# zju3dv/RelightableAvatar

Hardware: AMD Instinct MI355X
Metric: rays_per_sec (higher is better)
Workload: dtype f16

## Files before the change

relightableavatar_amd/csrc/ra_api.cpp:

```cpp
#include "ra_api_impl.hpp"
#include <cmath>

int check_ready(ra_ctx* c, const char* who) {
    if (!c) { ra_set_error(std::string(who) + ": null ctx"); return 1; }
    if (!c->have_weights) { ra_set_error(std::string(who) + ": weights not finalized"); return 1; }
    if (!c->have_frame) { ra_set_error(std::string(who) + ": no frame set (ra_set_frame)"); return 1; }
    if (hipSetDevice(c->device) != hipSuccess) { ra_set_error(std::string(who) + ": hipSetDevice failed"); return 1; }
    return 0;
}

static void zero_chunk_counters(ra_ctx* c, hipStream_t s) {
    hipMemsetAsync(icnt(c, 0), 0, CNT_ALL * sizeof(int), s);
    c->fc_next = 0;
    c->fc_wrapped = false;
    c->cnt_zero = true;
}
int* next_fine_counter(ra_ctx* c, hipStream_t s) {
    if (c->fc_next >= CNT_FC_SLOTS) {
        hipMemsetAsync(icnt(c, CNT_FC0), 0, CNT_FC_SLOTS * sizeof(int), s);
        c->fc_next = 0;
        c->fc_wrapped = true;
    }
    return icnt(c, CNT_FC0 + c->fc_next++);
}
// ... 329 lines not shown
    return 0;
}

struct LvisStage {
    const float *surf, *norm_slots, *acc, *bbox;
    const int *hit_idx, *hit_count;
    int P, no_visibility, local_visibility;
    float near_offset;
    const ra_trace_params* shadow;
    int n_boxes;
    const float* boxes;
    const int *box_start, *pix_nn, *perm;
    bool split_wide_groups;
    float *lvis, *ldot;
};
static int light_visibility_stage(ra_ctx* c, LvisStage& st, hipStream_t s) {
    const int P = st.P;
    const ra_trace_params& shadow = *st.shadow;
    int err = 0;
    const int L = c->n_lights;
    const size_t NR = (size_t)P * L;
    st.lvis = c->buf<float>("lv_lvis", NR, &err);
    st.ldot = c->buf<float>("lv_ldot", NR, &err);
    ShadowGen g{};
    g.surf = st.surf; g.norm = st.norm_slots; g.acc = st.acc; g.hit_idx = st.hit_idx; g.hit_count = st.hit_count; g.ldir = c->light_dir.as<float>();
    for (int k = 0; k < 6; ++k) g.bbox[k] = st.bbox[k];
    g.n_boxes = st.n_boxes > 1 ? st.n_boxes : 0;
    for (int j = 0; j < g.n_boxes; ++j) {
        for (int k = 0; k < 6; ++k) g.boxes[j][k] = st.boxes[6 * j + k];
        g.box_start[j] = st.box_start[j];
    }
    if (g.n_boxes) g.box_start[g.n_boxes] = st.box_start[g.n_boxes];
    g.perm = g.n_boxes ? st.perm : nullptr;
    g.near_offset = st.near_offset; g.L = L; g.no_visibility = st.no_visibility; g.local_visibility = st.local_visibility;
    g.split_wide_groups = st.split_wide_groups ? 1 : 0;
    g.lvis = st.lvis; g.ldot = st.ldot;
    g.ray_count = icnt(c, CNT_RAYS);
    const bool traced = !(st.no_visibility || st.local_visibility);
    TraceState sh{};
    float* ssdf = nullptr;
    if (traced) {
        g.ray_pix = c->buf<int>("lv_pix", NR, &err);
        g.ray_light = c->buf<int>("lv_light", NR, &err);
        g.ray_slot = c->buf<int>("lv_slot", NR, &err);
        g.near_ = c->buf<float>("lv_near", NR, &err);
        g.far_ = c->buf<float>("lv_far", NR, &err);
        sh = alloc_trace(c, "sh_", (int)NR, shadow.soft_shadow != 0, &err);
        ssdf = c->buf<float>("sh_sdf", NR, &err);
    }
    const bool keyed = traced && key_tier(c) && c->key_valid;
    const size_t NK = keyed ? (size_t)P * (size_t)(L < KEY_LIGHTS_MAX ? L : KEY_LIGHTS_MAX) : 0;
    if (err) return 1;
    if (c->gate && c->gate->armed) RA_HIP(hipStreamWaitEvent(s, c->gate->done, 0));
    launch_shadow_gen(g, P, s, c->cnt_zero);
    c->cnt_zero = false;
    if (traced) {
        sh.near_ = g.near_; sh.far_ = g.far_; sh.tan_i = c->light_sharp.as<float>(); sh.light = g.ray_light;
        launch_trace_init(sh, (int)NR, g.ray_count, shadow, s);
        RaySet r2{};
        r2.mode = 2; r2.o = st.surf; r2.t = sh.t; r2.pix = g.ray_pix; r2.light = g.ray_light; r2.ldir = c->light_dir.as<float>();
        r2.n_dev = g.ray_count;
        r2.skip = c->cfg.query_skip ? sh.stuck : nullptr;
        r2.nn_hint = c->buf<int>("lv_nn", NR * 3, &err);
        if (err) return 1;
        for (int it = 0; it < shadow.iters; ++it) {
            r2.hint_valid = it > 0;
            r2.hint_src = it == 0 ? st.pix_nn : nullptr;
            r2.hint_src_index = it == 0 ? g.ray_pix : nullptr;
            if (hdq_pass(c, r2, (int)NR, shadow.dist_th, 1, ssdf, s, Q_OTHER, keyed ? c->key_mask.as<unsigned char>() : nullptr, (int)NK)) return 1;
            launch_trace_update(sh, ssdf, (int)NR, g.ray_count, it, shadow, s);
        }
        launch_shadow_scatter(sh.occ, g.ray_slot, g.ray_count, (int)NR, st.lvis, s);
        launch_accumulate(g.ray_count, &dcnt(c)->n_shadow_rays, s);
    }
    if (c->gate) { RA_HIP(hipEventRecord(c->gate->done, s)); c->gate->armed = true; }
    return 0;
}

int ra_begin_render(ra_ctx* c) {
    RA_CHECK(c, "ra_begin_render: null ctx");
    c->call_no = 0;
    return 0;
}

int ra_set_key_probes(ra_ctx* c, const float* probes, int n, int ph, int pw, int accumulate, void* stream) {
    RA_CHECK(c && n >= 0 && (n == 0 || (probes && ph > 0 && pw > 0)), "ra_set_key_probes: bad arguments");
    if (n == 0) { c->key_external = false; c->key_valid = false; return 0; }
    RA_CHECK(c->have_weights && c->n_lights > 0, "ra_set_key_probes: needs the relight network's light set (ra_finalize_weights)");
    RA_HIP(hipSetDevice(c->device));
    const bool acc = accumulate && c->key_external && c->key_valid;
    c->key_external = true;
    if (!key_tier(c)) { c->key_valid = false; return 0; }
    if (c->key_mask.ensure((size_t)c->n_lights) || c->key_share.ensure((size_t)c->n_lights * sizeof(float))) return 1;
    launch_key_lights(probes, n, ph, pw, c->light_dir.as<float>(), c->light_area.as<float>(), c->n_lights, c->cfg.key_light_share, KEY_LIGHTS_MAX,
                      acc ? 1 : 0, c->key_share.as<float>(), c->key_mask.as<unsigned char>(), (hipStream_t)stream);
    c->key_valid = true;
    RA_HIP(hipGetLastError());
    return 0;
}

static int sort_hits(ra_ctx* c, const char* who, const float* surf, const float* acc, int P, const float* bbox, int* hit_idx, hipStream_t s) {
    int err = 0;
    const size_t tb = sort_hits_temp_bytes(P);
    unsigned* k0 = c->buf<unsigned>("hs_k0", P, &err);
    unsigned* k1 = c->buf<unsigned>("hs_k1", P, &err);
    int* v0 = c->buf<int>("hs_v0", P, &err);
    char* tmp = c->buf<char>("hs_tmp", tb + 16, &err);
    if (err) return 1;
    if (launch_sort_hits(surf, acc, P, bbox, k0, k1, v0, hit_idx, tmp, tb, s)) { ra_set_error(std::string(who) + ": radix sort failed"); return 1; }
    return 0;
}
static int sort_rays(ra_ctx* c, const char* who, const float** ray_o, const float** ray_d, const float** near_, const float** far_, int P,
                     const float* bbox, const int** perm, hipStream_t s) {
    int err = 0;
    const size_t tb = sort_hits_temp_bytes(P);
    unsigned* k0 = c->buf<unsigned>("hs_k0", P, &err);
    unsigned* k1 = c->buf<unsigned>("hs_k1", P, &err);
    int* v0 = c->buf<int>("hs_v0", P, &err);
    int* pm = c->buf<int>("rs_perm", P, &err);
    char* tmp = c->buf<char>("hs_tmp", tb + 16, &err);
    float* so = c->buf<float>("rs_o", (size_t)P * 3, &err);
    float* sd = c->buf<float>("rs_d", (size_t)P * 3, &err);
    float* sn = c->buf<float>("rs_n", P, &err);
    float* sf = c->buf<float>("rs_f", P, &err);
    if (err) return 1;
    const int rc = bbox ? launch_sort_rays(*ray_o, *ray_d, *near_, *far_, P, bbox, k0, k1, v0, pm, tmp, tb, so, sd, sn, sf, s)
// ... 261 lines not shown
```

relightableavatar_amd/csrc/ra_kernels.hpp:

```cpp
#pragma once
#include "ra_common.hpp"
#include "ra_lpips_pack.hpp"

struct RaySet {
    int mode;
    const float* x;
    const float* o;
    const float* d;
    const float* t;
    const int* pix;
    const int* light;
    const float* ldir;
    const int* n_dev;
    const unsigned char* skip;
    int* nn_hint;
    int hint_valid;
    const int* hint_src;
    const int* hint_src_index;
};

struct HdqOut {
    float* sdf;
    int* fine_count;
    int* fine_idx;
// ... 28 lines not shown
struct TraceState {
    float *t, *d0, *dt, *st, *ot, *cd, *occ, *off, *rlx;
    const float *near_, *far_;
    const float* tan_i;
    const int* light;
    unsigned char* stuck;
};
void launch_trace_init(const TraceState& ts, int n, const int* n_dev, const ra_trace_params& p, hipStream_t s);

void launch_trace_update(const TraceState& ts, const float* sdf, int n, const int* n_dev, int iter,
                         const ra_trace_params& p, hipStream_t s);

void launch_surface_finish(const float* ray_o, const float* ray_d, const float* st, const float* occ, int P, float* surf,
                           float* depth, float* acc, int* hit_idx, int* hit_count, hipStream_t s, int* slot_of_ray = nullptr,
                           bool counter_is_zero = false);
void launch_slot_index(const int* hit_idx, const int* hit_count, int P, int* slot_of_ray, hipStream_t s);
struct MapJob { const float* src; float* dst; int C; int premul; int src_full; };
constexpr int RA_MAX_MAP_JOBS = 16;
struct EmitMaps { MapJob job[RA_MAX_MAP_JOBS]; long long end[RA_MAX_MAP_JOBS]; int n_jobs; const int* slot_of_ray; const float* acc; const int* perm; int P; };
void launch_emit_maps(const EmitMaps& m, hipStream_t s);
void launch_surface_samples(const float* surf, const float* ray_d, const int* hit_idx, const int* hit_count, int P, int S,
                            float range, float* x, float* v, int* n_out, hipStream_t s);
struct SurfaceMaps {
    float *cpts, *bpts, *resd, *norm, *albedo, *rough, *rgb;
    float* valbedo;
};
void launch_surface_composite(const float* raw, int C, int S, const int* hit_count, int P, int relight, const ra_config& cfg,
                              const SurfaceMaps& m, hipStream_t s);

constexpr int RA_MAX_BOXES = 32;
struct ShadowGen {
    const float* surf;
    const float* norm;
    const float* acc;
    const int* hit_idx;
    const int* hit_count;
    const float* ldir;
    float bbox[6];
    int n_boxes;
    float boxes[RA_MAX_BOXES][6];
    int box_start[RA_MAX_BOXES + 1];
    const int* perm;
    float near_offset;
    int L;
    int no_visibility, local_visibility;
    int split_wide_groups;
    float* lvis;
    float* ldot;
    int* ray_pix;
    int* ray_light;
    int* ray_slot;
    float *near_, *far_;
    int* ray_count;
};
void launch_key_lights(const float* probes, int n, int ph, int pw, const float* ldir, const float* area, int L, float share, int kmax,
                       int accumulate, float* smax, unsigned char* key, hipStream_t s);
void launch_gather_shard_rays(const long long* idx, int n, const float* ro, const float* rd, const float* nr, const float* fr, float* so, float* sd,
                              float* sn, float* sf, hipStream_t s);
void launch_scatter_rows(const float* src, const long long* src_idx, const long long* dst_idx, long long n, int C, float* dst, hipStream_t s);
void launch_shadow_gen(const ShadowGen& g, int P, hipStream_t s, bool counter_is_zero = false);
void launch_debug_aabb(const float* o, const float* d, int n, const float* bbox6, float* nr, float* fr, hipStream_t s);
void launch_debug_brdf(const float* p2l, const float* p2c, const float* nrm, const float* alb, const float* rough, int L, int N, const ra_config& cfg,
                       float* out, hipStream_t s);
size_t sort_hits_temp_bytes(int P);
int launch_sort_hits(const float* surf, const float* acc, int P, const float* bbox_min, unsigned* keys_in, unsigned* keys_out,
                     int* vals_in, int* hit_idx_out, void* temp, size_t temp_bytes, hipStream_t s);
void launch_shadow_scatter(const float* occ, const int* ray_slot, const int* ray_count, int max_rays, float* lvis, hipStream_t s);

struct ShadeIn {
    const float* ray_o;
    const float* surf;
    const int* idx;
    const int* count;
    int n;
    const float *norm, *albedo, *rough;
    const float *lvis, *ldot;
    const float *light_xyz, *light_area;
    int L;
    const float* probes;
    int n_probes, ph, pw;
    int want_spec;
    float *rgb, *shade, *spec;
};
void launch_shade(const ShadeIn& in, const ra_config& cfg, hipStream_t s);

constexpr int SHADE_BWD_MAX_GRID = 768;
constexpr size_t SHADE_BWD_LDS_BYTES = 65536;
struct ShadeBwd {
    const float *ray_o, *surf, *norm, *albedo, *rough;
    const float* lvis;
    const float *light_xyz, *light_area; int L;
    const float* probes; int n_probes, ph, pw;
    const float* d_rgb;
    int P;
    float *d_albedo, *d_rough, *d_probes;
    float* slabs;
};
int shade_bwd_grid(int P);
int shade_bwd_probes_per_launch(int ph, int pw);
void launch_shade_bwd(const ShadeBwd& a, const ra_config& cfg, hipStream_t s);

constexpr int HEADS_PARAMS = 99332;
constexpr int HEADS_MAX_GRID = 128;
constexpr int HEADS_CHUNK = 32768;
constexpr size_t HEADS_TAPE_BYTES_PER_TILE = 163840;
constexpr size_t HEADS_W16_BYTES = 2 * 66048 * 2;
struct HeadsIO {
    const float *theta, *feat;
    int n;
    float *albedo, *rough;
    const float *d_albedo, *d_rough;
    float* d_theta;
    void* w16;
    unsigned* amax;
    void* tape;
    float* slabs;
};
int heads_grid(int n);
void launch_heads_forward(const HeadsIO& io, const ra_config& cfg, hipStream_t s);
void launch_heads_backward(const HeadsIO& io, const ra_config& cfg, hipStream_t s);
// ... 240 lines not shown
```

relightableavatar_amd/csrc/ra_trace.hip:

```cpp
#include "ra_kernels.hpp"
#include "ra_shade_dev.hpp"
#include <hipcub/hipcub.hpp>

namespace {

constexpr int TPB = 256;

__device__ __forceinline__ int live_count(const int* n_dev, int n) { return n_dev ? min(*n_dev, n) : n; }

__device__ __forceinline__ float linspace01(int s, int S) {
    if (S == 1) return 0.f;
    const float step = 1.f / (float)(S - 1);
    return (s < S / 2) ? (float)s * step : 1.f - (float)(S - 1 - s) * step;
}

__global__ void trace_init_kernel(TraceState ts, int n_launch, const int* n_dev, float offset, float relax) {
    const int i = blockIdx.x * TPB + threadIdx.x;
    if (i >= live_count(n_dev, n_launch)) return;
    const float nr = ts.near_[i], fr = ts.far_[i];
    ts.t[i] = nr;
    ts.d0[i] = 1e9f;
    ts.occ[i] = 1.f;
    if (ts.stuck) ts.stuck[i] = 0;
    if (ts.dt) ts.dt[i] = 1e9f;
    if (ts.st) ts.st[i] = fr;
    if (ts.ot) ts.ot[i] = fr;
    if (ts.cd) ts.cd[i] = 1e9f;
    if (ts.off) ts.off[i] = offset;
    if (ts.rlx) ts.rlx[i] = relax;
}

template <bool SOFT>
__global__ void trace_update_kernel(TraceState ts, const float* __restrict__ sdf, int n_launch, const int* n_dev, int iter,
                                    ra_trace_params p) {
    const int i = blockIdx.x * TPB + threadIdx.x;
    if (i >= live_count(n_dev, n_launch)) return;
    const float d1 = sdf[i];
    const float d0 = ts.d0[i];
    float t = ts.t[i];
    const float t_prev = t;
    float occ = ts.occ[i];
    const float nr = ts.near_[i], fr = ts.far_[i];
    float tan_i = p.tan_i;
    if (SOFT) {
        const float ti = ts.tan_i ? (ts.light ? ts.tan_i[ts.light[i]] : ts.tan_i[i]) : p.tan_i;
        tan_i = p.tan_i_multiplier * ti;
    }
    const float tan2 = (1.f / tan_i) * 2.f;
    float off = ts.off ? ts.off[i] : p.offset;
    float rlx = ts.rlx ? ts.rlx[i] : p.relax;
    float ot = ts.ot ? ts.ot[i] : 0.f;
    if (SOFT && p.clay_book && iter >= p.shadow_skip_iter) {
        const float dx0 = d0 + rlx * d0 + off;
        const float dx1 = d1 + rlx * d1 + off;
        const float dy = (dx1 * dx1) / (2.f * dx0);
        const float dx = (sqrtf(dx1 * dx1 - dy * dy) - off) / (1.f + rlx);
        const float den = fmaxf(fmaxf(t - dy, nr), p.eps);
        const float cls = fmaxf(dx, 0.f) / den / tan2;
        const bool msk = (cls < occ) && (dy < t) && (dx1 > 0.f) && (dx0 > 0.f) && (dx > 0.f) && (dy > 0.f) && (dy < dx0);
        if (msk) { ot = t - dy; occ = cls; }
    }
    if (iter >= p.shadow_skip_iter) {
        const float cls = fmaxf(d1, 0.f) / fmaxf(fmaxf(t, nr), p.eps) / tan2;
        if (cls < occ) { ot = t; occ = cls; }
    }
    if (!SOFT) {
        const float d1u = fabsf(d1), d0u = fabsf(d0);
        float st = ts.st[i], cd = ts.cd[i];
        const float dt = ts.dt[i];
        const float s0 = (d0 > 0.f) ? 1.f : ((d0 < 0.f) ? -1.f : 0.f);
        const float s1 = (d1 > 0.f) ? 1.f : ((d1 < 0.f) ? -1.f : 0.f);
        if (s0 != s1) {
            st = t - dt * fminf(fmaxf(d1u / (d0u + d1u + p.eps), 0.f), 1.f);
            off = 0.f;
            rlx = 0.f;
        }
        if (d1u < cd) { cd = d1u; st = t; }
        ts.st[i] = st;
        ts.cd[i] = cd;
        ts.off[i] = off;
        ts.rlx[i] = rlx;
    }
    const float dtn = d1 + rlx * d1 + off;
    t = t + dtn;
    t = fminf(t, fr);
    t = fmaxf(t, nr);
    if (ts.dt) ts.dt[i] = dtn;
    ts.t[i] = t;
    if (ts.stuck) ts.stuck[i] = (t == t_prev || (SOFT && occ == 0.f)) ? 1 : 0;
    ts.d0[i] = d1;
    ts.occ[i] = occ;
    if (ts.ot) ts.ot[i] = ot;
}

__global__ void surface_finish_kernel(const float* __restrict__ ro, const float* __restrict__ rd, const float* __restrict__ st,
                                      const float* __restrict__ occ, int P, float* __restrict__ surf, float* __restrict__ depth,
                                      float* __restrict__ acc, int* __restrict__ hit_idx, int* __restrict__ hit_count, int* __restrict__ slot_of_ray) {
    const int i = blockIdx.x * TPB + threadIdx.x;
    bool hit = false;
    if (i < P) {
        if (slot_of_ray) slot_of_ray[i] = -1;
        const float s = st[i];
        const float sx = ro[3 * i] + s * rd[3 * i], sy = ro[3 * i + 1] + s * rd[3 * i + 1], sz = ro[3 * i + 2] + s * rd[3 * i + 2];
        surf[3 * i] = sx; surf[3 * i + 1] = sy; surf[3 * i + 2] = sz;
        depth[i] = (sx - ro[3 * i]) / rd[3 * i];
        const float a = 1.f - occ[i];
        acc[i] = a;
        hit = a > 0.f;
    }
    const unsigned long long m = __ballot(hit);
    if (m == 0ull) return;
    const int lane = threadIdx.x & 63;
    int base = 0;
    if (lane == 0) base = atomicAdd(hit_count, __popcll(m));
    base = __shfl(base, 0);
    if (hit) hit_idx[base + __popcll(m & ((1ull << lane) - 1ull))] = i;
}

__device__ __forceinline__ unsigned expand10t(unsigned v) {
    v = (v * 0x00010001u) & 0xFF0000FFu;
    v = (v * 0x00000101u) & 0x0F00F00Fu;
    v = (v * 0x00000011u) & 0xC30C30C3u;
    v = (v * 0x00000005u) & 0x49249249u;
    return v;
}

__global__ void hit_keys_kernel(const float* __restrict__ surf, const float* __restrict__ acc, int P, float bx, float by, float bz,
                                unsigned* __restrict__ keys, int* __restrict__ vals) {
    const int i = blockIdx.x * TPB + threadIdx.x;
    if (i >= P) return;
    unsigned k = 0xffffffffu;
    if (acc[i] > 0.f) {
        const unsigned qx = (unsigned)fminf(fmaxf((surf[3 * i] - bx) * 256.f, 0.f), 1023.f);
        const unsigned qy = (unsigned)fminf(fmaxf((surf[3 * i + 1] - by) * 256.f, 0.f), 1023.f);
        const unsigned qz = (unsigned)fminf(fmaxf((surf[3 * i + 2] - bz) * 256.f, 0.f), 1023.f);
        k = (expand10t(qx) << 2) | (expand10t(qy) << 1) | expand10t(qz);
    }
    keys[i] = k;
    vals[i] = i;
}

__global__ void ray_keys_kernel(const float* __restrict__ ro, const float* __restrict__ rd, const float* __restrict__ nr, int P,
                                float bx, float by, float bz, const float* __restrict__ origin_dev, unsigned* __restrict__ keys,
                                int* __restrict__ vals) {
    const int i = blockIdx.x * TPB + threadIdx.x;
// ... 211 lines not shown
            if (g.no_visibility) lv = 1.f;
            else if (g.local_visibility) lv = ldot > 0.f ? 1.f : 0.f;
            else {
                const bool front = (ldot > 0.f) && (acc > 0.f);
                lv = 0.f;
                if (front) {
                    const float d[3] = {dx, dy, dz};
                    aabb_near_far(box, o, d, nr, fr);
                    nr = fmaxf(nr, g.near_offset);
                    fr = fmaxf(fr, g.near_offset);
                    trace = nr < fr;
                    lv = 1.f;
                }
            }
            t_ldot[lane][ll] = ldot;
            t_lvis[lane][ll] = lv;
        }
        nrv[round] = nr; frv[round] = fr;
        if (trace) tmask |= 1u << round;
        const unsigned long long m = __ballot(trace);
        if (lane == 0) { cnt[0][ll] = __popcll(m & 0xffffffffull); cnt[1][ll] = __popcll(m >> 32); }
    }
    __syncthreads();
    if (threadIdx.x == 0) {
        int tot = 0;
        if (halves) {
            for (int hf = 0; hf < 2; ++hf)
                for (int k = 0; k < NL; ++k) { const int c = cnt[hf][k]; cnt[hf][k] = tot; tot += c; }
        } else {
            for (int k = 0; k < NL; ++k) {
                const int c0 = cnt[0][k], c1 = cnt[1][k];
                cnt[0][k] = tot; cnt[1][k] = tot + c0; tot += c0 + c1;
            }
        }
        cnt[0][NL] = tot ? atomicAdd(g.ray_count, tot) : 0;
    }
    __syncthreads();
    const int gbase = cnt[0][NL];
#pragma unroll
    for (int round = 0; round < ROUNDS; ++round) {
        const int ll = round * (TPB / 64) + wv;
        const bool trace = (tmask >> round) & 1u;
        const unsigned long long m = __ballot(trace);
        if (trace) {
            const int hf = lane >> 5;
            const unsigned mh = hf ? (unsigned)(m >> 32) : (unsigned)m;
            const int s = gbase + cnt[hf][ll] + __popc(mh & ((1u << (lane & 31)) - 1u));
            const int l = lc * SG_LIGHTS + ll;
            g.ray_pix[s] = r;
            g.ray_light[s] = l;
            g.ray_slot[s] = h * g.L + l;
            g.near_[s] = nrv[round];
            g.far_[s] = frv[round];
        }
    }
    const int col = threadIdx.x & (SG_LIGHTS - 1), l = lc * SG_LIGHTS + col;
    for (int row = threadIdx.x / SG_LIGHTS; row < 64; row += TPB / SG_LIGHTS) {
        const int hh = grp * 64 + row;
        if (hh < nh && l < g.L) {
            g.ldot[(size_t)hh * g.L + l] = t_ldot[row][col];
            g.lvis[(size_t)hh * g.L + l] = t_lvis[row][col];
        }
    }
}

__global__ void shadow_scatter_kernel(const float* __restrict__ occ, const int* __restrict__ ray_slot, const int* __restrict__ ray_count,
                                      int max_rays, float* __restrict__ lvis) {
    const int i = blockIdx.x * TPB + threadIdx.x;
    if (i >= min(*ray_count, max_rays)) return;
    lvis[ray_slot[i]] = occ[i];
}

__global__ __launch_bounds__(TPB) void key_lights_kernel(const float* __restrict__ probes, int n, int ph, int pw, const float* __restrict__ ldir,
                                                         const float* __restrict__ area, int L, float share, int kmax, int accumulate,
                                                         float* __restrict__ smax, unsigned char* __restrict__ key) {
    extern __shared__ float kl_w[];
    __shared__ float red[TPB / 64];
    for (int q = 0; q < n; ++q) {
        const float* img = probes + (size_t)q * ph * pw * 3;
        float part = 0.f;
        for (int l = threadIdx.x; l < L; l += TPB) {
            const float d[3] = {ldir[3 * l], ldir[3 * l + 1], ldir[3 * l + 2]};
            float c[3];
            sample_probe(img, ph, pw, d, c);
            float w = (c[0] + c[1] + c[2]) * (1.f / 3.f) * area[l];
            w = w > 0.f ? w : 0.f;
            kl_w[l] = w;
            part += w;
        }
#pragma unroll
        for (int sh = 32; sh > 0; sh >>= 1) part += __shfl_xor(part, sh);
        if ((threadIdx.x & 63) == 0) red[threadIdx.x >> 6] = part;
        __syncthreads();
        float total = 0.f;
#pragma unroll
        for (int k = 0; k < TPB / 64; ++k) total += red[k];
        for (int l = threadIdx.x; l < L; l += TPB) {
            const float sh_l = total > 0.f ? kl_w[l] / total : 0.f;
            smax[l] = (q == 0 && !accumulate) ? sh_l : fmaxf(smax[l], sh_l);
        }
        __syncthreads();
    }
    for (int l = threadIdx.x; l < L; l += TPB) kl_w[l] = smax[l];
    __syncthreads();
    const float thr = fmaxf(share, 4.f / (float)L);
    for (int l = threadIdx.x; l < L; l += TPB) {
        const float w = kl_w[l];
        bool cand = w >= thr;
        if (cand) {
            int rank = 0;
            for (int j = 0; j < L; ++j) rank += (kl_w[j] > w) || (kl_w[j] == w && j < l);
            cand = rank < kmax;
        }
        key[l] = (unsigned char)cand;
    }
}

__global__ void debug_brdf_kernel(const float* __restrict__ p2l, const float* __restrict__ p2c, const float* __restrict__ nrm, const float* __restrict__ alb,
                                  const float* __restrict__ rough, int L, int N, ra_config cfg, float* __restrict__ out) {
    const int i = blockIdx.x * TPB + threadIdx.x;
    if (i >= L * N) return;
// ... 187 lines not shown
    __syncthreads();
    float pre = 1.f;
    for (int k = 0; k < g; ++k) pre *= tseg[k][j];
#pragma unroll
    for (int c = 0; c < 15; ++c) part[g][c][j] = o[c] * pre;
    part[g][15][j] = acc * pre;
    part[g][16][j] = depth * pre;
    __syncthreads();
    if (blockIdx.x * 64 + j >= P) return;
    const int w_ = perm ? perm[r] : r;
    float a_ = 0.f;
#pragma unroll
    for (int k = 0; k < VC_SEG; ++k) a_ += part[k][15][j];
    if (g == 15) {
        float d_ = 0.f;
#pragma unroll
        for (int k = 0; k < VC_SEG; ++k) d_ += part[k][16][j];
        if (out.acc) out.acc[w_] = a_;
        if (out.depth) out.depth[w_] = d_;
        return;
    }
    float v = 0.f;
#pragma unroll
    for (int k = 0; k < VC_SEG; ++k) v += part[k][g][j];
    v += (1.f - a_) * bg;
    float* dst = g < 3 ? out.cpts : (g < 6 ? out.bpts : (g < 9 ? out.resd : (g < 12 ? out.norm : out.rgb)));
    if (dst) dst[3 * w_ + g % 3] = v;
}

inline dim3 grid_for(long long n) { return dim3((unsigned)((n + TPB - 1) / TPB)); }

}

void launch_debug_aabb(const float* o, const float* d, int n, const float* bbox6, float* nr, float* fr, hipStream_t s) {
    if (n <= 0) return;
    Box6 b; for (int k = 0; k < 6; ++k) b.v[k] = bbox6[k];
    hipLaunchKernelGGL(debug_aabb_kernel, grid_for(n), dim3(TPB), 0, s, o, d, n, b, nr, fr);
}

void launch_debug_brdf(const float* p2l, const float* p2c, const float* nrm, const float* alb, const float* rough, int L, int N, const ra_config& cfg,
                       float* out, hipStream_t s) {
    if (L * N <= 0) return;
    hipLaunchKernelGGL(debug_brdf_kernel, grid_for((long long)L * N), dim3(TPB), 0, s, p2l, p2c, nrm, alb, rough, L, N, cfg, out);
}

void launch_trace_init(const TraceState& ts, int n, const int* n_dev, const ra_trace_params& p, hipStream_t s) {
    if (n <= 0) return;
    hipLaunchKernelGGL(trace_init_kernel, grid_for(n), dim3(TPB), 0, s, ts, n, n_dev, p.offset, p.relax);
}

void launch_trace_update(const TraceState& ts, const float* sdf, int n, const int* n_dev, int iter, const ra_trace_params& p,
                         hipStream_t s) {
    if (n <= 0) return;
    if (p.soft_shadow) hipLaunchKernelGGL(trace_update_kernel<true>, grid_for(n), dim3(TPB), 0, s, ts, sdf, n, n_dev, iter, p);
    else hipLaunchKernelGGL(trace_update_kernel<false>, grid_for(n), dim3(TPB), 0, s, ts, sdf, n, n_dev, iter, p);
}

void launch_surface_finish(const float* ray_o, const float* ray_d, const float* st, const float* occ, int P, float* surf,
                           float* depth, float* acc, int* hit_idx, int* hit_count, hipStream_t s, int* slot_of_ray, bool counter_is_zero) {
    if (!counter_is_zero) hipMemsetAsync(hit_count, 0, sizeof(int), s);
    if (P <= 0) return;
    hipLaunchKernelGGL(surface_finish_kernel, grid_for(P), dim3(TPB), 0, s, ray_o, ray_d, st, occ, P, surf, depth, acc, hit_idx, hit_count, slot_of_ray);
}

void launch_slot_index(const int* hit_idx, const int* hit_count, int P, int* slot_of_ray, hipStream_t s) {
    if (P <= 0) return;
    hipLaunchKernelGGL(slot_index_kernel, grid_for(P), dim3(TPB), 0, s, hit_idx, hit_count, slot_of_ray);
}

void launch_emit_maps(const EmitMaps& m, hipStream_t s) {
    if (m.n_jobs <= 0 || m.P <= 0) return;
    hipLaunchKernelGGL(emit_maps_kernel, grid_for(m.end[m.n_jobs - 1]), dim3(TPB), 0, s, m);
}

void launch_surface_samples(const float* surf, const float* ray_d, const int* hit_idx, const int* hit_count, int P, int S,
                            float range, float* x, float* v, int* n_out, hipStream_t s) {
    if (P <= 0) { hipMemsetAsync(n_out, 0, sizeof(int), s); return; }
    hipLaunchKernelGGL(surface_samples_kernel, grid_for((long long)P * S), dim3(TPB), 0, s, surf, ray_d, hit_idx, hit_count, S, range, x, v, n_out);
}

void launch_surface_composite(const float* raw, int C, int S, const int* hit_count, int P, int relight, const ra_config& cfg,
                              const SurfaceMaps& m, hipStream_t s) {
    if (P <= 0) return;
    hipLaunchKernelGGL(surface_composite_kernel, grid_for(P), dim3(TPB), 0, s, raw, C, S, hit_count, relight, cfg, m);
}

void launch_key_lights(const float* probes, int n, int ph, int pw, const float* ldir, const float* area, int L, float share, int kmax,
                       int accumulate, float* smax, unsigned char* key, hipStream_t s) {
    hipLaunchKernelGGL(key_lights_kernel, dim3(1), dim3(TPB), (size_t)L * sizeof(float), s, probes, n, ph, pw, ldir, area, L, share, kmax, accumulate, smax, key);
}

void launch_light_dirs(const float* xyz, int L, float* ldir, hipStream_t s) {
    hipLaunchKernelGGL(light_dirs_kernel, grid_for(L), dim3(TPB), 0, s, xyz, L, ldir);
}

void launch_shadow_gen(const ShadowGen& g, int P, hipStream_t s, bool counter_is_zero) {
    if (!counter_is_zero) hipMemsetAsync(g.ray_count, 0, sizeof(int), s);
    if (P <= 0) return;
    const long long groups = ((long long)P + 63) / 64;
    const int lchunks = (g.L + SG_LIGHTS - 1) / SG_LIGHTS;
    hipLaunchKernelGGL(shadow_gen_kernel, dim3((unsigned)(groups * lchunks)), dim3(TPB), 0, s, g);
}

__global__ void ground_hit_kernel(GroundIn g, float* __restrict__ t_out, float* __restrict__ surf, float* __restrict__ depth,
                                  float* __restrict__ norm_slots, int* __restrict__ hit_idx, int* __restrict__ hit_count) {
    const int i = blockIdx.x * TPB + threadIdx.x;
    bool hit = false;
// ... 410 lines not shown
    nr = t_near / nd / nd;
    fr = t_far / nd / nd;
    return t_near < t_far;
}

__global__ void ray_mask_kernel(RayCam c, unsigned char* __restrict__ mask) {
    const int i = blockIdx.x * TPB + threadIdx.x;
    if (i >= c.H * c.W) return;
    float o[3], d[3], nr, fr;
    mask[i] = pixel_ray(c, i, o, d, nr, fr) ? 1 : 0;
}

__global__ void ray_emit_kernel(RayCam c, const int* __restrict__ pix_idx, const int* __restrict__ count, float* __restrict__ ro,
                                float* __restrict__ rd, float* __restrict__ near_, float* __restrict__ far_) {
    const int i = blockIdx.x * TPB + threadIdx.x;
    if (i >= *count) return;
    float o[3], d[3], nr, fr;
    pixel_ray(c, pix_idx[i], o, d, nr, fr);
#pragma unroll
    for (int k = 0; k < 3; ++k) { ro[3 * i + k] = o[k]; rd[3 * i + k] = d[k]; }
    near_[i] = nr;
    far_[i] = fr;
}

size_t gen_rays_temp_bytes(int n) {
    size_t bytes = 0;
    hipcub::DeviceSelect::Flagged(nullptr, bytes, hipcub::CountingInputIterator<int>(0), (const unsigned char*)nullptr, (int*)nullptr, (int*)nullptr, n);
    return bytes;
}

int launch_gen_rays(const RayCam& cam, unsigned char* mask, int* pix_idx, int* count_dev, void* temp, size_t temp_bytes,
                    float* ray_o, float* ray_d, float* near, float* far, hipStream_t s) {
    const int n = cam.H * cam.W;
    if (n <= 0) { hipMemsetAsync(count_dev, 0, sizeof(int), s); return 0; }
    hipLaunchKernelGGL(ray_mask_kernel, grid_for(n), dim3(TPB), 0, s, cam, mask);
    if (hipcub::DeviceSelect::Flagged(temp, temp_bytes, hipcub::CountingInputIterator<int>(0), mask, pix_idx, count_dev, n, s) != hipSuccess) return 1;
    hipLaunchKernelGGL(ray_emit_kernel, grid_for(n), dim3(TPB), 0, s, cam, pix_idx, count_dev, ray_o, ray_d, near, far);
    return 0;
}

size_t sort_hits_temp_bytes(int P) {
    size_t bytes = 0;
    hipcub::DeviceRadixSort::SortPairs(nullptr, bytes, (const unsigned*)nullptr, (unsigned*)nullptr, (const int*)nullptr, (int*)nullptr, P);
    return bytes;
}

int launch_sort_hits(const float* surf, const float* acc, int P, const float* bbox_min, unsigned* keys_in, unsigned* keys_out,
                     int* vals_in, int* hit_idx_out, void* temp, size_t temp_bytes, hipStream_t s) {
    if (P <= 0) return 0;
    hipLaunchKernelGGL(hit_keys_kernel, grid_for(P), dim3(TPB), 0, s, surf, acc, P, bbox_min[0], bbox_min[1], bbox_min[2], keys_in, vals_in);
    return hipcub::DeviceRadixSort::SortPairs(temp, temp_bytes, keys_in, keys_out, vals_in, hit_idx_out, P, 0, 32, s) == hipSuccess ? 0 : 1;
}

void launch_shadow_scatter(const float* occ, const int* ray_slot, const int* ray_count, int max_rays, float* lvis, hipStream_t s) {
    if (max_rays <= 0) return;
    hipLaunchKernelGGL(shadow_scatter_kernel, grid_for(max_rays), dim3(TPB), 0, s, occ, ray_slot, ray_count, max_rays, lvis);
}

void launch_shade(const ShadeIn& in, const ra_config& cfg, hipStream_t s) {
    if (in.n <= 0) return;
    hipLaunchKernelGGL(shade_kernel, grid_for((long long)in.n * 64), dim3(TPB), 0, s, in, cfg);
}

void launch_scatter_maps(const int* hit_idx, const int* hit_count, int P, int premultiply, const float* acc_full, const float* src,
                         int C, float* dst, int src_full, const int* perm, hipStream_t s) {
    if (P <= 0) return;
    hipLaunchKernelGGL(scatter_maps_kernel, grid_for((long long)P * C), dim3(TPB), 0, s, hit_idx, hit_count, premultiply, acc_full, src, C, dst, src_full, perm);
}

int launch_sort_rays(const float* ro, const float* rd, const float* nr, const float* fr, int P, const float* bbox_min, unsigned* keys_in,
                     unsigned* keys_out, int* vals_in, int* perm, void* temp, size_t temp_bytes, float* so, float* sd, float* sn, float* sf,
                     hipStream_t s, float near_min, float far_max) {
    if (P <= 0) return 0;
    float* origin_dev = nullptr;
    if (!bbox_min) {
        origin_dev = reinterpret_cast<float*>(keys_out);
        hipLaunchKernelGGL(entry_min_kernel, dim3(1), dim3(1024), 0, s, ro, rd, nr, P, origin_dev);
    }
    hipLaunchKernelGGL(ray_keys_kernel, grid_for(P), dim3(TPB), 0, s, ro, rd, nr, P, bbox_min ? bbox_min[0] : 0.f, bbox_min ? bbox_min[1] : 0.f,
                       bbox_min ? bbox_min[2] : 0.f, origin_dev, keys_in, vals_in);
    if (hipcub::DeviceRadixSort::SortPairs(temp, temp_bytes, keys_in, keys_out, vals_in, perm, P, 0, 32, s) != hipSuccess) return 1;
    hipLaunchKernelGGL(gather_rays_kernel, grid_for(P), dim3(TPB), 0, s, perm, P, ro, rd, nr, fr, so, sd, sn, sf, near_min, far_max);
    return 0;
}

void launch_gather_shard_rays(const long long* idx, int n, const float* ro, const float* rd, const float* nr, const float* fr, float* so, float* sd,
                              float* sn, float* sf, hipStream_t s) {
    if (n <= 0) return;
    hipLaunchKernelGGL(gather_shard_rays_kernel, grid_for(n), dim3(TPB), 0, s, idx, n, ro, rd, nr, fr, so, sd, sn, sf);
}

void launch_scatter_rows(const float* src, const long long* src_idx, const long long* dst_idx, long long n, int C, float* dst, hipStream_t s) {
    if (n <= 0) return;
    hipLaunchKernelGGL(scatter_rows_kernel, grid_for(n * C), dim3(TPB), 0, s, src, src_idx, dst_idx, n, C, dst);
}

void launch_accumulate(const int* count, unsigned long long* dst, hipStream_t s) {
    hipLaunchKernelGGL(accumulate_kernel, dim3(1), dim3(1), 0, s, count, dst);
}

void launch_gather_rows(const int* hit_idx, const int* hit_count, int P, const float* src, int C, float* dst, hipStream_t s) {
    if (P <= 0) return;
    hipLaunchKernelGGL(gather_rows_kernel, grid_for((long long)P * C), dim3(TPB), 0, s, hit_idx, hit_count, src, C, dst);
}

__global__ void iota_kernel(int* __restrict__ idx, int n, int* __restrict__ count) {
    const int i = blockIdx.x * TPB + threadIdx.x;
    if (i == 0 && count) *count = n;
    if (i < n) idx[i] = i;
// ... 72 lines not shown
```

Before: 9.135 million.

## Fuse trace init into shadow gen, vectorize soft trace update, fold accumulate

Shadow-ray trace state is now initialised inside the shadow generation kernel, so the separate trace_init launch and its pass over every ray slot go away. The shadow ray-count accumulation moves into the scatter kernel, which removes one more launch. The soft-shadow trace update now handles four rays per thread with float4 loads and stores when the pointers are aligned, cutting the thread count and widening memory transactions. This adds alignment-dependent branching and duplicated init logic, and the init now runs only for generated slots rather than across the whole launch range.

```diff
diff --git a/relightableavatar_amd/csrc/ra_api.cpp b/relightableavatar_amd/csrc/ra_api.cpp
--- a/relightableavatar_amd/csrc/ra_api.cpp
+++ b/relightableavatar_amd/csrc/ra_api.cpp
@@ -405,11 +405,13 @@
     const size_t NK = keyed ? (size_t)P * (size_t)(L < KEY_LIGHTS_MAX ? L : KEY_LIGHTS_MAX) : 0;
     if (err) return 1;
     if (c->gate && c->gate->armed) RA_HIP(hipStreamWaitEvent(s, c->gate->done, 0));
+    if (traced) {
+        sh.near_ = g.near_; sh.far_ = g.far_; sh.tan_i = c->light_sharp.as<float>(); sh.light = g.ray_light;
+        g.init = sh; g.init_offset = shadow.offset; g.init_relax = shadow.relax;
+    }
     launch_shadow_gen(g, P, s, c->cnt_zero);
     c->cnt_zero = false;
     if (traced) {
-        sh.near_ = g.near_; sh.far_ = g.far_; sh.tan_i = c->light_sharp.as<float>(); sh.light = g.ray_light;
-        launch_trace_init(sh, (int)NR, g.ray_count, shadow, s);
         RaySet r2{};
         r2.mode = 2; r2.o = st.surf; r2.t = sh.t; r2.pix = g.ray_pix; r2.light = g.ray_light; r2.ldir = c->light_dir.as<float>();
         r2.n_dev = g.ray_count;
@@ -423,8 +425,7 @@
             if (hdq_pass(c, r2, (int)NR, shadow.dist_th, 1, ssdf, s, Q_OTHER, keyed ? c->key_mask.as<unsigned char>() : nullptr, (int)NK)) return 1;
             launch_trace_update(sh, ssdf, (int)NR, g.ray_count, it, shadow, s);
         }
-        launch_shadow_scatter(sh.occ, g.ray_slot, g.ray_count, (int)NR, st.lvis, s);
-        launch_accumulate(g.ray_count, &dcnt(c)->n_shadow_rays, s);
+        launch_shadow_scatter(sh.occ, g.ray_slot, g.ray_count, (int)NR, st.lvis, &dcnt(c)->n_shadow_rays, s);
     }
     if (c->gate) { RA_HIP(hipEventRecord(c->gate->done, s)); c->gate->armed = true; }
     return 0;
diff --git a/relightableavatar_amd/csrc/ra_kernels.hpp b/relightableavatar_amd/csrc/ra_kernels.hpp
--- a/relightableavatar_amd/csrc/ra_kernels.hpp
+++ b/relightableavatar_amd/csrc/ra_kernels.hpp
@@ -104,6 +104,8 @@
     int* ray_slot;
     float *near_, *far_;
     int* ray_count;
+    TraceState init;
+    float init_offset, init_relax;
 };
 void launch_key_lights(const float* probes, int n, int ph, int pw, const float* ldir, const float* area, int L, float share, int kmax,
                        int accumulate, float* smax, unsigned char* key, hipStream_t s);
@@ -117,7 +119,8 @@
 size_t sort_hits_temp_bytes(int P);
 int launch_sort_hits(const float* surf, const float* acc, int P, const float* bbox_min, unsigned* keys_in, unsigned* keys_out,
                      int* vals_in, int* hit_idx_out, void* temp, size_t temp_bytes, hipStream_t s);
-void launch_shadow_scatter(const float* occ, const int* ray_slot, const int* ray_count, int max_rays, float* lvis, hipStream_t s);
+void launch_shadow_scatter(const float* occ, const int* ray_slot, const int* ray_count, int max_rays, float* lvis, unsigned long long* total,
+                           hipStream_t s);
 
 struct ShadeIn {
     const float* ray_o;
diff --git a/relightableavatar_amd/csrc/ra_trace.hip b/relightableavatar_amd/csrc/ra_trace.hip
--- a/relightableavatar_amd/csrc/ra_trace.hip
+++ b/relightableavatar_amd/csrc/ra_trace.hip
@@ -30,26 +30,22 @@
     if (ts.rlx) ts.rlx[i] = relax;
 }
 
+struct RayStep { float d1, d0, t, occ, nr, fr, ti, off, rlx, ot, st, cd, dt; unsigned char stuck; };
+
 template <bool SOFT>
-__global__ void trace_update_kernel(TraceState ts, const float* __restrict__ sdf, int n_launch, const int* n_dev, int iter,
-                                    ra_trace_params p) {
-    const int i = blockIdx.x * TPB + threadIdx.x;
-    if (i >= live_count(n_dev, n_launch)) return;
-    const float d1 = sdf[i];
-    const float d0 = ts.d0[i];
-    float t = ts.t[i];
+__device__ __forceinline__ void trace_update_ray(RayStep& r, int iter, const ra_trace_params& p) {
+    const float d1 = r.d1;
+    const float d0 = r.d0;
+    float t = r.t;
     const float t_prev = t;
-    float occ = ts.occ[i];
-    const float nr = ts.near_[i], fr = ts.far_[i];
+    float occ = r.occ;
+    const float nr = r.nr, fr = r.fr;
     float tan_i = p.tan_i;
-    if (SOFT) {
-        const float ti = ts.tan_i ? (ts.light ? ts.tan_i[ts.light[i]] : ts.tan_i[i]) : p.tan_i;
-        tan_i = p.tan_i_multiplier * ti;
-    }
+    if (SOFT) tan_i = p.tan_i_multiplier * r.ti;
     const float tan2 = (1.f / tan_i) * 2.f;
-    float off = ts.off ? ts.off[i] : p.offset;
-    float rlx = ts.rlx ? ts.rlx[i] : p.relax;
-    float ot = ts.ot ? ts.ot[i] : 0.f;
+    float off = r.off;
+    float rlx = r.rlx;
+    float ot = r.ot;
     if (SOFT && p.clay_book && iter >= p.shadow_skip_iter) {
         const float dx0 = d0 + rlx * d0 + off;
         const float dx1 = d1 + rlx * d1 + off;
@@ -66,8 +62,8 @@
     }
     if (!SOFT) {
         const float d1u = fabsf(d1), d0u = fabsf(d0);
-        float st = ts.st[i], cd = ts.cd[i];
-        const float dt = ts.dt[i];
+        float st = r.st, cd = r.cd;
+        const float dt = r.dt;
         const float s0 = (d0 > 0.f) ? 1.f : ((d0 < 0.f) ? -1.f : 0.f);
         const float s1 = (d1 > 0.f) ? 1.f : ((d1 < 0.f) ? -1.f : 0.f);
         if (s0 != s1) {
@@ -76,21 +72,97 @@
             rlx = 0.f;
         }
         if (d1u < cd) { cd = d1u; st = t; }
-        ts.st[i] = st;
-        ts.cd[i] = cd;
-        ts.off[i] = off;
-        ts.rlx[i] = rlx;
+        r.st = st;
+        r.cd = cd;
+        r.off = off;
+        r.rlx = rlx;
     }
     const float dtn = d1 + rlx * d1 + off;
     t = t + dtn;
     t = fminf(t, fr);
     t = fmaxf(t, nr);
-    if (ts.dt) ts.dt[i] = dtn;
-    ts.t[i] = t;
-    if (ts.stuck) ts.stuck[i] = (t == t_prev || (SOFT && occ == 0.f)) ? 1 : 0;
-    ts.d0[i] = d1;
-    ts.occ[i] = occ;
-    if (ts.ot) ts.ot[i] = ot;
+    r.dt = dtn;
+    r.t = t;
+    r.stuck = (t == t_prev || (SOFT && occ == 0.f)) ? 1 : 0;
+    r.d0 = d1;
+    r.occ = occ;
+    r.ot = ot;
+}
+
+template <bool SOFT>
+__device__ __forceinline__ void trace_update_one(const TraceState& ts, const float* __restrict__ sdf, int i, int iter, const ra_trace_params& p) {
+    RayStep r;
+    r.d1 = sdf[i];
+    r.d0 = ts.d0[i];
+    r.t = ts.t[i];
+    r.occ = ts.occ[i];
+    r.nr = ts.near_[i]; r.fr = ts.far_[i];
+    r.ti = 0.f;
+    if (SOFT) r.ti = ts.tan_i ? (ts.light ? ts.tan_i[ts.light[i]] : ts.tan_i[i]) : p.tan_i;
+    r.off = ts.off ? ts.off[i] : p.offset;
+    r.rlx = ts.rlx ? ts.rlx[i] : p.relax;
+    r.ot = ts.ot ? ts.ot[i] : 0.f;
+    r.st = r.cd = r.dt = 0.f;
+    if (!SOFT) { r.st = ts.st[i]; r.cd = ts.cd[i]; r.dt = ts.dt[i]; }
+    trace_update_ray<SOFT>(r, iter, p);
+    if (!SOFT) { ts.st[i] = r.st; ts.cd[i] = r.cd; ts.off[i] = r.off; ts.rlx[i] = r.rlx; }
+    if (ts.dt) ts.dt[i] = r.dt;
+    ts.t[i] = r.t;
+    if (ts.stuck) ts.stuck[i] = r.stuck;
+    ts.d0[i] = r.d0;
+    ts.occ[i] = r.occ;
+    if (ts.ot) ts.ot[i] = r.ot;
+}
+
+constexpr int TU_RAYS = 4;
+template <bool SOFT>
+__global__ void trace_update_kernel(TraceState ts, const float* __restrict__ sdf, int n_launch, const int* n_dev, int iter,
+                                    ra_trace_params p) {
+    const int n = live_count(n_dev, n_launch);
+    if (!SOFT) {
+        const int i = blockIdx.x * TPB + threadIdx.x;
+        if (i >= n) return;
+        trace_update_one<false>(ts, sdf, i, iter, p);
+        return;
+    }
+    const long long i0l = ((long long)blockIdx.x * TPB + threadIdx.x) * TU_RAYS;
+    if (i0l >= n) return;
+    const int i0 = (int)i0l;
+    auto low = [](const void* q) { return (unsigned)reinterpret_cast<size_t>(q); };
+    const bool vec = ts.tan_i && ts.light && ts.ot && ts.stuck && !ts.dt && !ts.off && !ts.rlx &&
+                     ((low(sdf) | low(ts.d0) | low(ts.t) | low(ts.occ) | low(ts.ot) | low(ts.near_) | low(ts.far_) | low(ts.light)) & 15u) == 0u &&
+                     (low(ts.stuck) & 3u) == 0u;
+    if (!vec || i0 + TU_RAYS > n) {
+        for (int i = i0; i < min(i0 + TU_RAYS, n); ++i) trace_update_one<true>(ts, sdf, i, iter, p);
+        return;
+    }
+    const int q = i0 / TU_RAYS;
+    const float4 v_d1 = reinterpret_cast<const float4*>(sdf)[q], v_d0 = reinterpret_cast<const float4*>(ts.d0)[q];
+    const float4 v_t = reinterpret_cast<const float4*>(ts.t)[q], v_occ = reinterpret_cast<const float4*>(ts.occ)[q];
+    const float4 v_nr = reinterpret_cast<const float4*>(ts.near_)[q], v_fr = reinterpret_cast<const float4*>(ts.far_)[q];
+    const float4 v_ot = reinterpret_cast<const float4*>(ts.ot)[q];
+    const int4 v_l = reinterpret_cast<const int4*>(ts.light)[q];
+    const float a_d1[4] = {v_d1.x, v_d1.y, v_d1.z, v_d1.w}, a_d0[4] = {v_d0.x, v_d0.y, v_d0.z, v_d0.w};
+    const float a_t[4] = {v_t.x, v_t.y, v_t.z, v_t.w}, a_occ[4] = {v_occ.x, v_occ.y, v_occ.z, v_occ.w};
+    const float a_nr[4] = {v_nr.x, v_nr.y, v_nr.z, v_nr.w}, a_fr[4] = {v_fr.x, v_fr.y, v_fr.z, v_fr.w};
+    const float a_ot[4] = {v_ot.x, v_ot.y, v_ot.z, v_ot.w};
+    const int a_l[4] = {v_l.x, v_l.y, v_l.z, v_l.w};
+    float ti[4];
+#pragma unroll
+    for (int k = 0; k < 4; ++k) ti[k] = ts.tan_i[a_l[k]];
+    RayStep r[4];
+#pragma unroll
+    for (int k = 0; k < 4; ++k) {
+        r[k].d1 = a_d1[k]; r[k].d0 = a_d0[k]; r[k].t = a_t[k]; r[k].occ = a_occ[k]; r[k].nr = a_nr[k]; r[k].fr = a_fr[k]; r[k].ti = ti[k];
+        r[k].off = p.offset; r[k].rlx = p.relax; r[k].ot = a_ot[k];
+        r[k].st = r[k].cd = r[k].dt = 0.f;
+        trace_update_ray<true>(r[k], iter, p);
+    }
+    reinterpret_cast<float4*>(ts.t)[q] = make_float4(r[0].t, r[1].t, r[2].t, r[3].t);
+    reinterpret_cast<unsigned*>(ts.stuck)[q] = (unsigned)r[0].stuck | ((unsigned)r[1].stuck << 8) | ((unsigned)r[2].stuck << 16) | ((unsigned)r[3].stuck << 24);
+    reinterpret_cast<float4*>(ts.d0)[q] = make_float4(r[0].d0, r[1].d0, r[2].d0, r[3].d0);
+    reinterpret_cast<float4*>(ts.occ)[q] = make_float4(r[0].occ, r[1].occ, r[2].occ, r[3].occ);
+    reinterpret_cast<float4*>(ts.ot)[q] = make_float4(r[0].ot, r[1].ot, r[2].ot, r[3].ot);
 }
 
 __global__ void surface_finish_kernel(const float* __restrict__ ro, const float* __restrict__ rd, const float* __restrict__ st,
@@ -408,6 +480,17 @@
             g.ray_slot[s] = h * g.L + l;
             g.near_[s] = nrv[round];
             g.far_[s] = frv[round];
+            const TraceState& ts = g.init;
+            ts.t[s] = nrv[round];
+            ts.d0[s] = 1e9f;
+            ts.occ[s] = 1.f;
+            if (ts.stuck) ts.stuck[s] = 0;
+            if (ts.dt) ts.dt[s] = 1e9f;
+            if (ts.st) ts.st[s] = frv[round];
+            if (ts.ot) ts.ot[s] = frv[round];
+            if (ts.cd) ts.cd[s] = 1e9f;
+            if (ts.off) ts.off[s] = g.init_offset;
+            if (ts.rlx) ts.rlx[s] = g.init_relax;
         }
     }
     const int col = threadIdx.x & (SG_LIGHTS - 1), l = lc * SG_LIGHTS + col;
@@ -421,8 +504,9 @@
 }
 
 __global__ void shadow_scatter_kernel(const float* __restrict__ occ, const int* __restrict__ ray_slot, const int* __restrict__ ray_count,
-                                      int max_rays, float* __restrict__ lvis) {
+                                      int max_rays, float* __restrict__ lvis, unsigned long long* __restrict__ total) {
     const int i = blockIdx.x * TPB + threadIdx.x;
+    if (i == 0) atomicAdd(total, (unsigned long long)*ray_count);
     if (i >= min(*ray_count, max_rays)) return;
     lvis[ray_slot[i]] = occ[i];
 }
@@ -716,7 +800,7 @@
 void launch_trace_update(const TraceState& ts, const float* sdf, int n, const int* n_dev, int iter, const ra_trace_params& p,
                          hipStream_t s) {
     if (n <= 0) return;
-    if (p.soft_shadow) hipLaunchKernelGGL(trace_update_kernel<true>, grid_for(n), dim3(TPB), 0, s, ts, sdf, n, n_dev, iter, p);
+    if (p.soft_shadow) hipLaunchKernelGGL(trace_update_kernel<true>, grid_for(((long long)n + TU_RAYS - 1) / TU_RAYS), dim3(TPB), 0, s, ts, sdf, n, n_dev, iter, p);
     else hipLaunchKernelGGL(trace_update_kernel<false>, grid_for(n), dim3(TPB), 0, s, ts, sdf, n, n_dev, iter, p);
 }
 
@@ -1233,9 +1317,10 @@
     return hipcub::DeviceRadixSort::SortPairs(temp, temp_bytes, keys_in, keys_out, vals_in, hit_idx_out, P, 0, 32, s) == hipSuccess ? 0 : 1;
 }
 
-void launch_shadow_scatter(const float* occ, const int* ray_slot, const int* ray_count, int max_rays, float* lvis, hipStream_t s) {
+void launch_shadow_scatter(const float* occ, const int* ray_slot, const int* ray_count, int max_rays, float* lvis, unsigned long long* total,
+                           hipStream_t s) {
     if (max_rays <= 0) return;
-    hipLaunchKernelGGL(shadow_scatter_kernel, grid_for(max_rays), dim3(TPB), 0, s, occ, ray_slot, ray_count, max_rays, lvis);
+    hipLaunchKernelGGL(shadow_scatter_kernel, grid_for(max_rays), dim3(TPB), 0, s, occ, ray_slot, ray_count, max_rays, lvis, total);
 }
 
 void launch_shade(const ShadeIn& in, const ra_config& cfg, hipStream_t s) {
```

New measurement: 9.132 million (median of 2 runs). Within noise of the previous version (-0.0%).
